# Champii/raiko

Hardware: AMD Instinct MI355X
Metric: proven RISC-V cycles/sec (higher is better)
Workload: dtype u32 (BabyBear Montgomery)

## Files before the change

### raiko_amd/csrc/internal.hpp

```cpp
#pragma once
#include <hip/hip_runtime.h>

#include <cstring>
#include <map>
#include <memory>
#include <new>
#include <string>
#include <unordered_map>
#include <vector>

#include "../../include/raiko_hip.h"
#include "taps.hpp"
#include "bb.hpp"
#include "ntt_core.hpp"
#include "poseidon2_core.hpp"
#include "params.hpp"

struct rk_ctx {
    int device = 0;
    hipStream_t stream = nullptr;
    bool own_stream = false;
    std::string last_error;

    uint32_t* d_tables = nullptr;
// ... 79 lines not shown
int ntt_reverse_from(rk_ctx* ctx, uint32_t* d_dst, const uint32_t* d_src, size_t size, size_t count, bool fuse_zk_shift);
int ntt_forward(rk_ctx* ctx, uint32_t* d_out, const uint32_t* d_in, size_t in_size, size_t count,
                unsigned expand_bits);
int zk_shift(rk_ctx* ctx, uint32_t* d_io, size_t size, size_t count);
int bit_reverse(rk_ctx* ctx, uint32_t* d_io, size_t size, size_t count);

int hash_rows(rk_ctx* ctx, uint32_t* d_out, const uint32_t* d_matrix, size_t rows, size_t cols);
int hash_fold(rk_ctx* ctx, uint32_t* d_nodes, size_t output_size);
int merkle_build(rk_ctx* ctx, uint32_t* d_nodes, const uint32_t* d_matrix, size_t rows, size_t cols);
int pow_grind(rk_ctx* ctx, const uint32_t* h_cells, unsigned bits, uint32_t* nonce);
int duplex_grind(rk_ctx* ctx, const uint32_t* h_state, const uint32_t* h_input, unsigned n_input, unsigned bits, uint32_t* witness);

int eltwise_add(rk_ctx* ctx, uint32_t* d_out, const uint32_t* a, const uint32_t* b, size_t n);
int eltwise_sum_ext(rk_ctx* ctx, uint32_t* d_out, const uint32_t* d_in, size_t count, size_t to_add);
int eltwise_zeroize(rk_ctx* ctx, uint32_t* d_io, size_t n);
int fri_fold(rk_ctx* ctx, uint32_t* d_out, const uint32_t* d_in, size_t out_count, const bb::Ext& mix);
int fri_fold_evals(rk_ctx* ctx, uint32_t* d_out_ext, const uint32_t* d_in_ext, size_t n_out, const bb::Ext& beta);
int gather_sample(rk_ctx* ctx, uint32_t* d_dst, const uint32_t* d_src, size_t idx, size_t size, size_t stride);
int gather_rows(rk_ctx* ctx, uint32_t* d_dst, const uint32_t* d_matrix, size_t rows, size_t cols,
                const uint32_t* d_idx, size_t n_idx);
int gather_digests(rk_ctx* ctx, uint32_t* d_dst, const uint32_t* d_nodes, const uint32_t* d_idx, size_t n_idx);
struct GatherJob {
    const uint32_t* matrix;
    const uint32_t* nodes;
    uint64_t rows, cols, idx_off, dst_off;
    uint32_t n, path_len;
};
int gather_many(rk_ctx* ctx, uint32_t* d_dst, const uint32_t* d_idx, const GatherJob* d_jobs, const GatherJob* h_jobs, size_t n_jobs);
int ext_powers(rk_ctx* ctx, uint32_t* d_pw_ext, const bb::Ext& x, size_t n, bool bit_reversed);
int ext_powers_many(rk_ctx* ctx, uint32_t* d_pw_ext, const bb::Ext* h_pts, size_t n_pts, size_t n, bool bit_reversed);
int bit_reverse_ext(rk_ctx* ctx, uint32_t* d_io_ext, size_t size, size_t count);
constexpr size_t HASH_FOLD_TOP_MAX = 4096;
int hash_fold_top(rk_ctx* ctx, uint32_t* d_nodes, size_t top_output_size);
int eval_dot(rk_ctx* ctx, uint32_t* d_out_ext, const uint32_t* d_coeffs, size_t size, const uint32_t* d_which,
             const uint32_t* d_pw_ext, const uint32_t* d_pw_sel, size_t eval_count);
int mix_poly_coeffs(rk_ctx* ctx, uint32_t* d_out_ext, const bb::Ext& mix_start, const bb::Ext& mix,
                    const uint32_t* d_in, const uint32_t* h_combos, size_t input_size, size_t count);
int poly_divide(rk_ctx* ctx, uint32_t* d_poly_ext, size_t count, const bb::Ext& z, bb::Ext* h_rem);
int poly_divide_many(rk_ctx* ctx, uint32_t* d_base_ext, size_t count, const size_t* h_offsets, const bb::Ext* h_z,
                     size_t n_items, bb::Ext* h_rems, uint32_t* d_rems = nullptr);
int prefix_products(rk_ctx* ctx, uint32_t* d_io_ext, size_t count);
int scatter(rk_ctx* ctx, uint32_t* d_into, size_t into_words, const uint32_t* h_index, size_t n_cycles,
            const uint32_t* h_offsets, const uint32_t* h_values);
int program_eval_check(const rk_program* prog, const rk_circuit_view* view, const uint32_t poly_mix[4], uint32_t* d_check);
int program_poly_ext(const rk_program* prog, uint32_t wm, const uint32_t poly_mix[4], const uint32_t* eval_u_ext, size_t n_taps,
                     const uint32_t* globals, uint32_t n_globals, const uint32_t* mix, uint32_t n_mix, uint32_t out_ext[4]);
int pcs_coset_lde_rows(rk_ctx* ctx, uint32_t* d_out, const uint32_t* d_in, size_t h, size_t w, uint32_t** keep_cols = nullptr);
int pcs_cols_to_rows_bitrev(rk_ctx* ctx, uint32_t* d_out, const uint32_t* d_cols, size_t H, size_t w);
int pcs_eval_at(rk_ctx* ctx, uint32_t* d_out_ext, const uint32_t* d_lde, size_t H, size_t w, const uint32_t* h_points, size_t n_points,
                bool cols = false);
int pcs_reduce_openings(rk_ctx* ctx, uint32_t* d_ro_ext, const uint32_t* d_lde, size_t H, size_t w, size_t n_points,
                        const uint32_t* h_points, const uint32_t* h_ys, const bb::Ext& alpha, uint64_t alpha_offset, bool cols = false);
int pcs_coset_lde_cols(rk_ctx* ctx, uint32_t* d_cols, const uint32_t* d_in, size_t h, size_t w);
int ext_sub_at(rk_ctx* ctx, uint32_t* d_ext, const uint32_t* h_idx, const bb::Ext* h_delta, size_t n);
void p3_release_pools();

struct CodeKey {
    uint32_t fp[4];
    uint32_t po2, cols, blowup_log2, queries;
    uint32_t root27m, shiftm;
    uint32_t p2[8];
    bool operator==(const CodeKey& o) const { return std::memcmp(this, &o, sizeof(CodeKey)) == 0; }
};
struct CodeEntry {
    CodeKey key{};
    int device = 0;
    uint32_t* coeffs = nullptr;
    uint32_t* evaluated = nullptr;
    uint32_t* nodes = nullptr;
    std::vector<uint32_t> top;
// ... 16 lines not shown
```

### raiko_amd/csrc/kernels_poly.hip

```cpp
#include "internal.hpp"

#include <algorithm>
#include <cstring>

namespace {

using bb::Ext;
constexpr int TPB = 256;

inline unsigned grid_for(size_t n, unsigned cap = 16384) {
    size_t b = (n + TPB - 1) / TPB;
    if (b < 1) b = 1;
    return (unsigned)(b > cap ? cap : b);
}

__device__ __forceinline__ Ext load_ext(const uint32_t* p) {
    uint4 v = *reinterpret_cast<const uint4*>(p);
    return Ext{{v.x, v.y, v.z, v.w}};
}
__device__ __forceinline__ void store_ext(uint32_t* p, const Ext& e) {
    *reinterpret_cast<uint4*>(p) = make_uint4(e.c[0], e.c[1], e.c[2], e.c[3]);
}

__global__ void add_kernel(uint32_t* out, const uint32_t* a, const uint32_t* b, size_t n) {
    size_t i = (size_t)blockIdx.x * blockDim.x + threadIdx.x, st = (size_t)gridDim.x * blockDim.x;
    for (; i < n; i += st) out[i] = bb::add(a[i], b[i]);
}
__global__ void zeroize_kernel(uint32_t* io, size_t n) {
    size_t i = (size_t)blockIdx.x * blockDim.x + threadIdx.x, st = (size_t)gridDim.x * blockDim.x;
    for (; i < n; i += st)
        if (io[i] == bb::INVALID) io[i] = 0;
}
__global__ void sum_ext_kernel(uint32_t* out, const uint32_t* in, size_t count, size_t to_add) {
    size_t i = (size_t)blockIdx.x * blockDim.x + threadIdx.x, st = (size_t)gridDim.x * blockDim.x;
    for (; i < count; i += st) {
        Ext tot = bb::ext_zero();
        for (size_t j = 0; j < to_add; j++) tot = bb::add(tot, load_ext(in + (j * count + i) * 4));
#pragma unroll
        for (int k = 0; k < 4; k++) out[(size_t)k * count + i] = tot.c[k];
    }
}

struct FoldPows {
    Ext p[16];
};
template <int LOG_A>
__global__ void fri_fold_kernel(uint32_t* out, const uint32_t* in, size_t count, FoldPows pw, uint32_t wm) {
    constexpr unsigned A = 1u << LOG_A;
    size_t idx = (size_t)blockIdx.x * blockDim.x + threadIdx.x, st = (size_t)gridDim.x * blockDim.x;
    for (; idx < count; idx += st) {
        Ext tot = bb::ext_zero();
// ... 65 lines not shown
        store_ext(pw + pos * 4, cur);
        cur = bb::mul(cur, x, wm);
    }
}
__global__ void ext_powers_many_kernel(uint32_t* pw, const Ext* xs, size_t n, unsigned rev_bits, uint32_t wm) {
    size_t t = (size_t)blockIdx.x * blockDim.x + threadIdx.x;
    size_t start = t * PW_CH;
    if (start >= n) return;
    const Ext x = xs[blockIdx.y];
    pw += (size_t)blockIdx.y * n * 4;
    Ext cur = bb::pow(x, (uint64_t)start, wm);
    size_t end = start + PW_CH < n ? start + PW_CH : n;
    for (size_t k = start; k < end; k++) {
        size_t pos = rev_bits ? (size_t)bb::bitrev((uint32_t)k, rev_bits) : k;
        store_ext(pw + pos * 4, cur);
        cur = bb::mul(cur, x, wm);
    }
}
__global__ void bit_reverse_ext_kernel(uint32_t* io, size_t total, size_t size, unsigned bits) {
    size_t idx = (size_t)blockIdx.x * blockDim.x + threadIdx.x, st = (size_t)gridDim.x * blockDim.x;
    for (; idx < total; idx += st) {
        uint32_t pos = (uint32_t)(idx & (size - 1));
        uint32_t rev = bb::bitrev(pos, bits);
        if (pos < rev) {
            size_t other = idx - pos + rev;
            Ext a = load_ext(io + idx * 4), b = load_ext(io + other * 4);
            store_ext(io + idx * 4, b);
            store_ext(io + other * 4, a);
        }
    }
}

constexpr int DOT_BLOCKS = 64;
__global__ __launch_bounds__(TPB) void eval_dot_kernel(uint32_t* __restrict__ partial, const uint32_t* __restrict__ coeffs,
                                                       size_t size, const uint32_t* __restrict__ which,
                                                       const uint32_t* __restrict__ pw, const uint32_t* __restrict__ sel) {
    __shared__ uint32_t red[TPB * 4];
    size_t e = blockIdx.y;
    const uint32_t* c = coeffs + (size_t)which[e] * size;
    const uint32_t* p = pw + (size_t)sel[e] * size * 4;
    Ext acc = bb::ext_zero();
    constexpr size_t STEP = (size_t)DOT_BLOCKS * TPB;
    size_t k = (size_t)blockIdx.x * TPB + threadIdx.x;
    for (; k + 3 * STEP < size; k += 4 * STEP) {
        uint32_t v[4];
        Ext t[4];
#pragma unroll
        for (int u = 0; u < 4; u++) {
            v[u] = c[k + u * STEP];
            t[u] = load_ext(p + (k + u * STEP) * 4);
        }
#pragma unroll
        for (int u = 0; u < 4; u++) acc = bb::add(acc, bb::scale(t[u], v[u]));
    }
    for (; k < size; k += STEP) acc = bb::add(acc, bb::scale(load_ext(p + k * 4), c[k]));
#pragma unroll
    for (int j = 0; j < 4; j++) red[threadIdx.x * 4 + j] = acc.c[j];
    __syncthreads();
    for (int s = TPB / 2; s > 0; s >>= 1) {
        if ((int)threadIdx.x < s) {
#pragma unroll
            for (int j = 0; j < 4; j++)
                red[threadIdx.x * 4 + j] = bb::add(red[threadIdx.x * 4 + j], red[(threadIdx.x + s) * 4 + j]);
        }
        __syncthreads();
    }
    if (threadIdx.x < 4) partial[(e * DOT_BLOCKS + blockIdx.x) * 4 + threadIdx.x] = red[threadIdx.x];
}
__global__ void eval_reduce_kernel(uint32_t* out, const uint32_t* partial, size_t n_eval) {
    size_t i = (size_t)blockIdx.x * blockDim.x + threadIdx.x;
    if (i >= n_eval * 4) return;
    size_t e = i >> 2, j = i & 3;
    uint32_t acc = 0;
    for (int b = 0; b < DOT_BLOCKS; b++) acc = bb::add(acc, partial[(e * DOT_BLOCKS + b) * 4 + j]);
    out[i] = acc;
}

__global__ void mix_kernel(uint32_t* __restrict__ out, const uint32_t* __restrict__ in, size_t count,
                           const uint32_t* __restrict__ slot_combo, const uint32_t* __restrict__ slot_off,
                           const uint32_t* __restrict__ cols, const uint32_t* __restrict__ pows) {
    constexpr unsigned U = 8;
    unsigned slot = blockIdx.y;
    size_t combo = slot_combo[slot];
    unsigned t0 = slot_off[slot], t1 = slot_off[slot + 1];
    size_t idx = (size_t)blockIdx.x * blockDim.x + threadIdx.x, st = (size_t)gridDim.x * blockDim.x;
    for (; idx < count; idx += st) {
        uint32_t* o = out + (combo * count + idx) * 4;
        Ext acc = load_ext(o);
        unsigned t = t0;
        for (; t + U <= t1; t += U) {
            uint32_t v[U];
#pragma unroll
            for (unsigned u = 0; u < U; u++) v[u] = in[(size_t)cols[t + u] * count + idx];
#pragma unroll
            for (unsigned u = 0; u < U; u++) acc = bb::add(acc, bb::scale(load_ext(pows + (size_t)(t + u) * 4), v[u]));
        }
        for (; t < t1; t++) {
            Ext pw = load_ext(pows + (size_t)t * 4);
            acc = bb::add(acc, bb::scale(pw, in[(size_t)cols[t] * count + idx]));
        }
        store_ext(o, acc);
    }
}

constexpr int DIV_CH = 64;
constexpr int DIV_NT = 1024;
constexpr int DIV_GRP = 32;
struct DivItem {
    Ext z, zL;
    unsigned long long off;
    uint32_t wm;
    uint32_t pad_;
};
__global__ void div_tops_kernel(uint32_t* tops, const uint32_t* base, size_t count, size_t nchunks, const DivItem* items) {
    size_t b = (size_t)blockIdx.x * blockDim.x + threadIdx.x;
    if (b >= nchunks) return;
    const DivItem it = items[blockIdx.y];
    const uint32_t* poly = base + it.off * 4;
    size_t start = b * DIV_CH;
    size_t end = start + DIV_CH < count ? start + DIV_CH : count;
    Ext s = bb::ext_zero();
    for (size_t k = end; k-- > start;) s = bb::add(bb::mul(s, it.z, it.wm), load_ext(poly + k * 4));
    store_ext(tops + ((size_t)blockIdx.y * nchunks + b) * 4, s);
}
__global__ __launch_bounds__(DIV_NT) void div_carry_kernel(uint32_t* carry, const uint32_t* tops, size_t nchunks,
                                                           const DivItem* items, uint32_t* rem_out) {
    __shared__ uint32_t seg[DIV_NT * 4];
    __shared__ uint32_t sup[DIV_GRP * 4];
    const unsigned t = threadIdx.x;
    const DivItem it = items[blockIdx.y];
    tops += (size_t)blockIdx.y * nchunks * 4;
    carry += (size_t)blockIdx.y * nchunks * 4;
    const size_t per = (nchunks + DIV_NT - 1) / DIV_NT;
    const size_t s0 = (size_t)t * per, s1 = s0 + per < nchunks ? s0 + per : nchunks;
// ... 156 lines not shown
    }
    return RK_OK;
}
int ext_powers(rk_ctx* ctx, uint32_t* d_pw_ext, const bb::Ext& x, size_t n, bool bit_reversed) {
    if (n == 0) return RK_OK;
    if (bit_reversed && !is_pow2(n)) return RK_ERR_INVALID;
    size_t lanes = (n + PW_CH - 1) / PW_CH;
    KTimer kt(ctx, RK_KCLASS_POLY, (double)n * 16);
    hipLaunchKernelGGL(ext_powers_kernel, dim3((unsigned)((lanes + TPB - 1) / TPB)), dim3(TPB), 0, ctx->stream, d_pw_ext,
                       x, n, bit_reversed ? log2u(n) : 0u, ctx->sys.wm);
    return post_launch(ctx, "ext_powers_kernel");
}
int ext_powers_many(rk_ctx* ctx, uint32_t* d_pw_ext, const bb::Ext* h_pts, size_t n_pts, size_t n, bool bit_reversed) {
    if (n == 0 || n_pts == 0) return RK_OK;
    if ((bit_reversed && !is_pow2(n)) || n_pts > 65535) return RK_ERR_INVALID;
    void* d = nullptr;
    RK_TRY(scratch(ctx, n_pts * 16, &d));
    RK_TRY(upload(ctx, d, h_pts, n_pts * 16));
    size_t lanes = (n + PW_CH - 1) / PW_CH;
    KTimer kt(ctx, RK_KCLASS_POLY, (double)n * 16 * n_pts);
    hipLaunchKernelGGL(ext_powers_many_kernel, dim3((unsigned)((lanes + TPB - 1) / TPB), (unsigned)n_pts), dim3(TPB), 0, ctx->stream,
                       d_pw_ext, (const Ext*)d, n, bit_reversed ? log2u(n) : 0u, ctx->sys.wm);
    return post_launch(ctx, "ext_powers_many_kernel");
}
int bit_reverse_ext(rk_ctx* ctx, uint32_t* d_io_ext, size_t size, size_t count) {
    if (!is_pow2(size) || count == 0) return RK_ERR_INVALID;
    if (size <= 2) return RK_OK;
    size_t total = size * count;
    KTimer kt(ctx, RK_KCLASS_BIT_REVERSE, (double)total * 32);
    hipLaunchKernelGGL(bit_reverse_ext_kernel, dim3(grid_for(total)), dim3(TPB), 0, ctx->stream, d_io_ext, total, size,
                       log2u(size));
    return post_launch(ctx, "bit_reverse_ext_kernel");
}
int eval_dot(rk_ctx* ctx, uint32_t* d_out_ext, const uint32_t* d_coeffs, size_t size, const uint32_t* d_which,
             const uint32_t* d_pw_ext, const uint32_t* d_pw_sel, size_t eval_count) {
    if (eval_count == 0) return RK_OK;
    if (eval_count > 65535) return RK_ERR_INVALID;
    void* partial = nullptr;
    RK_TRY(dev_alloc(ctx, eval_count * DOT_BLOCKS * 16, &partial));
    KTimer kt(ctx, RK_KCLASS_POLY, (double)eval_count * size * 20);
    hipLaunchKernelGGL(eval_dot_kernel, dim3(DOT_BLOCKS, (unsigned)eval_count), dim3(TPB), 0, ctx->stream,
                       (uint32_t*)partial, d_coeffs, size, d_which, d_pw_ext, d_pw_sel);
    int st = post_launch(ctx, "eval_dot_kernel");
    if (st == RK_OK) {
        hipLaunchKernelGGL(eval_reduce_kernel, dim3((unsigned)((eval_count * 4 + TPB - 1) / TPB)), dim3(TPB), 0,
                           ctx->stream, d_out_ext, (const uint32_t*)partial, eval_count);
        st = post_launch(ctx, "eval_reduce_kernel");
    }
    dev_free(ctx, partial);
    return st;
}

int mix_poly_coeffs(rk_ctx* ctx, uint32_t* d_out_ext, const bb::Ext& mix_start, const bb::Ext& mix,
                    const uint32_t* d_in, const uint32_t* h_combos, size_t input_size, size_t count) {
    if (input_size == 0 || count == 0) return RK_OK;
    std::vector<uint32_t> order(input_size);
    for (size_t i = 0; i < input_size; i++) order[i] = (uint32_t)i;
    std::stable_sort(order.begin(), order.end(), [&](uint32_t a, uint32_t b) { return h_combos[a] < h_combos[b]; });
    std::vector<bb::Ext> pw(input_size);
    bb::Ext cur = mix_start;
    for (size_t i = 0; i < input_size; i++) {
        pw[i] = cur;
        cur = bb::mul(cur, mix, ctx->sys.wm);
    }
    std::vector<uint32_t> slot_combo, slot_off, cols(input_size), pows(input_size * 4);
    for (size_t t = 0; t < input_size; t++) {
        uint32_t i = order[t];
        if (t == 0 || h_combos[i] != h_combos[order[t - 1]]) {
            slot_combo.push_back(h_combos[i]);
            slot_off.push_back((uint32_t)t);
        }
        cols[t] = i;
        std::memcpy(&pows[t * 4], pw[i].c, 16);
    }
    slot_off.push_back((uint32_t)input_size);
    size_t n_slots = slot_combo.size();
    size_t o_combo = 0, o_off = o_combo + n_slots, o_cols = o_off + n_slots + 1;
    size_t o_pows = (o_cols + input_size + 3) & ~(size_t)3;
    size_t words = o_pows + input_size * 4;
    std::vector<uint32_t> pack(words, 0);
    std::memcpy(&pack[o_combo], slot_combo.data(), n_slots * 4);
    std::memcpy(&pack[o_off], slot_off.data(), (n_slots + 1) * 4);
    std::memcpy(&pack[o_cols], cols.data(), input_size * 4);
    std::memcpy(&pack[o_pows], pows.data(), input_size * 16);
    void* d = nullptr;
    RK_TRY(scratch(ctx, words * 4, &d));
    RK_TRY(upload(ctx, d, pack.data(), words * 4));
    const uint32_t* dp = (const uint32_t*)d;
    KTimer kt(ctx, RK_KCLASS_POLY, (double)count * (input_size * 4 + n_slots * 32));
    hipLaunchKernelGGL(mix_kernel, dim3(grid_for(count, 4096), (unsigned)n_slots), dim3(TPB), 0, ctx->stream, d_out_ext,
                       d_in, count, dp + o_combo, dp + o_off, dp + o_cols, dp + o_pows);
    return post_launch(ctx, "mix_kernel");
}

int poly_divide_many(rk_ctx* ctx, uint32_t* d_base_ext, size_t count, const size_t* h_offsets, const bb::Ext* h_z,
                     size_t n_items, bb::Ext* h_rems, uint32_t* d_rems) {
    if (count == 0 || n_items == 0 || n_items > 65535) return RK_ERR_INVALID;
    size_t nchunks = (count + DIV_CH - 1) / DIV_CH;
    if (nchunks > (size_t)DIV_NT * 4096) return RK_ERR_INVALID;
    std::vector<DivItem> items(n_items);
    for (size_t i = 0; i < n_items; i++) {
        items[i].z = h_z[i];
        items[i].zL = bb::pow(h_z[i], (uint64_t)DIV_CH, ctx->sys.wm);
        items[i].off = h_offsets[i];
        items[i].wm = ctx->sys.wm;
        items[i].pad_ = 0;
    }
    void* buf = nullptr;
    size_t items_bytes = (n_items * sizeof(DivItem) + 15) & ~(size_t)15;
    RK_TRY(dev_alloc(ctx, items_bytes + n_items * (2 * nchunks + 1) * 16, &buf));
    DivItem* d_items = (DivItem*)buf;
    uint32_t* tops = (uint32_t*)((char*)buf + items_bytes);
    uint32_t* carry = tops + n_items * nchunks * 4;
    uint32_t* rem = carry + n_items * nchunks * 4;
    int st = RK_OK;
    do {
        hipError_t e = hipSuccess;
        st = upload(ctx, d_items, items.data(), n_items * sizeof(DivItem));
        if (st != RK_OK) break;
        unsigned blocks = (unsigned)((nchunks + TPB - 1) / TPB);
        KTimer kt(ctx, RK_KCLASS_POLY, (double)count * 48 * n_items);
        hipLaunchKernelGGL(div_tops_kernel, dim3(blocks, (unsigned)n_items), dim3(TPB), 0, ctx->stream, tops, d_base_ext,
                           count, nchunks, d_items);
        st = post_launch(ctx, "div_tops_kernel");
// ... 94 lines not shown
    bb::Ext b{{beta[0], beta[1], beta[2], beta[3]}};
    return rk::fri_fold_evals(ctx, d_out_ext, d_in_ext, n_out, b);
    RK_GUARD_END
}
int rk_gather_sample(rk_ctx* ctx, uint32_t* d_dst, const uint32_t* d_src, size_t idx, size_t size, size_t stride) {
    RK_GUARD_BEGIN
    if (!ctx || (size && (!d_dst || !d_src))) return RK_ERR_INVALID;
    RK_HIP_TRY(ctx, hipSetDevice(ctx->device));
    return rk::gather_sample(ctx, d_dst, d_src, idx, size, stride);
    RK_GUARD_END
}

int rk_batch_evaluate_any(rk_ctx* ctx, const uint32_t* d_coeffs, size_t poly_count, size_t size,
                          const uint32_t* h_which, const uint32_t* h_xs, size_t eval_count, uint32_t* h_out) {
    RK_GUARD_BEGIN
    if (!ctx || !d_coeffs || !is_pow2(size)) return RK_ERR_INVALID;
    if (eval_count == 0) return RK_OK;
    if (!h_which || !h_xs || !h_out) return RK_ERR_INVALID;
    for (size_t e = 0; e < eval_count; e++)
        if (h_which[e] >= poly_count) return RK_ERR_INVALID;
    RK_HIP_TRY(ctx, hipSetDevice(ctx->device));
    std::vector<bb::Ext> pts;
    std::vector<uint32_t> sel(eval_count);
    for (size_t e = 0; e < eval_count; e++) {
        bb::Ext x{{h_xs[e * 4], h_xs[e * 4 + 1], h_xs[e * 4 + 2], h_xs[e * 4 + 3]}};
        size_t j = 0;
        for (; j < pts.size(); j++)
            if (bb::eq(pts[j], x)) break;
        if (j == pts.size()) pts.push_back(x);
        sel[e] = (uint32_t)j;
    }
    void *d_pw = nullptr, *d_small = nullptr;
    RK_TRY(rk::dev_alloc(ctx, pts.size() * size * 16, &d_pw));
    int st = rk::dev_alloc(ctx, eval_count * (4 + 4 + 16) + 32, &d_small);
    if (st != RK_OK) {
        rk::dev_free(ctx, d_pw);
        return st;
    }
    uint32_t* d_which = (uint32_t*)d_small;
    uint32_t* d_sel = d_which + eval_count;
    uint32_t* d_out = d_sel + eval_count;
    if (((uintptr_t)d_out & 15) != 0) d_out += (16 - ((uintptr_t)d_out & 15)) / 4;
    do {
        hipError_t e1 = hipMemcpyAsync(d_which, h_which, eval_count * 4, hipMemcpyHostToDevice, ctx->stream);
        hipError_t e2 = hipMemcpyAsync(d_sel, sel.data(), eval_count * 4, hipMemcpyHostToDevice, ctx->stream);
        if (e1 != hipSuccess || e2 != hipSuccess) { st = RK_ERR_HIP; ctx->last_error = "evaluate_any h2d"; break; }
        for (size_t j = 0; j < pts.size() && st == RK_OK; j++)
            st = rk::ext_powers(ctx, (uint32_t*)d_pw + j * size * 4, pts[j], size, false);
        if (st != RK_OK) break;
        st = rk::eval_dot(ctx, d_out, d_coeffs, size, d_which, (const uint32_t*)d_pw, d_sel, eval_count);
        if (st != RK_OK) break;
        hipError_t e3 = hipMemcpyAsync(h_out, d_out, eval_count * 16, hipMemcpyDeviceToHost, ctx->stream);
        if (e3 == hipSuccess) e3 = hipStreamSynchronize(ctx->stream);
        if (e3 != hipSuccess) { st = RK_ERR_HIP; ctx->last_error = "evaluate_any d2h"; }
    } while (0);
    if (st != RK_OK) (void)hipStreamSynchronize(ctx->stream);
    rk::dev_free(ctx, d_small);
    rk::dev_free(ctx, d_pw);
    return st;
    RK_GUARD_END
}

int rk_mix_poly_coeffs(rk_ctx* ctx, uint32_t* d_out_ext, const uint32_t mix_start[4], const uint32_t mix[4],
                       const uint32_t* d_in, const uint32_t* h_combos, size_t input_size, size_t count) {
    RK_GUARD_BEGIN
    if (!ctx || !d_out_ext || !d_in || !h_combos || !mix_start || !mix) return RK_ERR_INVALID;
    RK_HIP_TRY(ctx, hipSetDevice(ctx->device));
    bb::Ext ms{{mix_start[0], mix_start[1], mix_start[2], mix_start[3]}};
    bb::Ext mx{{mix[0], mix[1], mix[2], mix[3]}};
    return rk::mix_poly_coeffs(ctx, d_out_ext, ms, mx, d_in, h_combos, input_size, count);
    RK_GUARD_END
}

int rk_poly_divide(rk_ctx* ctx, uint32_t* d_polys_ext, size_t count, const uint32_t z[4], uint32_t* h_rem) {
    RK_GUARD_BEGIN
    if (!ctx || !d_polys_ext || !z || count == 0) return RK_ERR_INVALID;
    RK_HIP_TRY(ctx, hipSetDevice(ctx->device));
    bb::Ext zz{{z[0], z[1], z[2], z[3]}};
    bb::Ext rem;
    RK_TRY(rk::poly_divide(ctx, d_polys_ext, count, zz, &rem));
    if (h_rem) std::memcpy(h_rem, rem.c, 16);
    return RK_OK;
    RK_GUARD_END
}

}
```

### raiko_amd/csrc/prover.hip

```cpp
#include "internal.hpp"

#include <algorithm>
#include <cstring>
#include <memory>

namespace {

using bb::Ext;

struct Transcript {
    p2::Rng rng;
    std::vector<uint32_t> proof;
    explicit Transcript(const p2::Any* kc) : rng(kc) {}
    void write(const uint32_t* w, size_t n) { proof.insert(proof.end(), w, w + n); }
    void commit(const uint32_t* digest) { rng.mix(digest); }
    uint32_t random_elem() { return rng.random_elem(); }
    Ext random_ext() { return rng.random_ext(); }
    uint32_t random_bits(unsigned bits) { return rng.random_bits(bits); }
};

struct DevBuf {
    rk_ctx* ctx = nullptr;
    void* p = nullptr;
    bool borrowed = false;
// ... 459 lines not shown
        if (taps.combo_backs[b] > max_back) max_back = taps.combo_backs[b];
    if (max_back > 64) return RK_ERR_INVALID;
    size_t n_pts = (size_t)max_back + 2;
    std::vector<Ext> pts(n_pts);
    for (uint32_t b = 0; b <= max_back; b++) pts[b] = bb::scale(z, bb::pow(back_one, b));
    pts[max_back + 1] = z_pow;
    std::vector<Ext> all_xs(tot_taps), coeff_u(tot_taps + CHECK_SIZE);
    {
        DevBuf d_pw, d_small;
        RK_TRY(d_pw.alloc(ctx, n_pts * N * 16));
        RK_TRY(rk::ext_powers_many(ctx, d_pw.u32(), pts.data(), n_pts, N, true));
        std::vector<Ext> eval_u(tot_taps + CHECK_SIZE);
        std::vector<uint32_t> which, sel;
        std::vector<size_t> first(5, 0);
        size_t pos = 0;
        uint32_t reg = 0;
        for (uint32_t gid = 0; gid < 3; gid++) {
            for (; reg < taps.n_regs && taps.reg_group[reg] == gid; reg++) {
                uint32_t cb = taps.reg_combo[reg];
                for (uint32_t b = taps.combo_off[cb]; b < taps.combo_off[cb + 1]; b++) {
                    which.push_back(taps.reg_offset[reg]);
                    sel.push_back(taps.combo_backs[b]);
                    all_xs[pos++] = pts[taps.combo_backs[b]];
                }
            }
            first[gid + 1] = pos;
        }
        for (uint32_t i = 0; i < CHECK_SIZE; i++) {
            which.push_back(i);
            sel.push_back(max_back + 1);
        }
        first[4] = pos + CHECK_SIZE;
        const size_t n_ev = first[4];
        RK_TRY(d_small.alloc(ctx, n_ev * (4 + 4 + 16) + 32));
        uint32_t* d_which = d_small.u32();
        uint32_t* d_sel = d_which + n_ev;
        uint32_t* d_out = d_sel + n_ev;
        if (((uintptr_t)d_out & 15) != 0) d_out += (16 - ((uintptr_t)d_out & 15)) / 4;
        RK_TRY(rk::upload(ctx, d_which, which.data(), n_ev * 4));
        RK_TRY(rk::upload(ctx, d_sel, sel.data(), n_ev * 4));
        for (uint32_t gid = 0; gid < 4; gid++) {
            const PolyGroup& pg = gid < 3 ? groups[gid] : check;
            const size_t a = first[gid], n = first[gid + 1] - a;
            if (n) RK_TRY(rk::eval_dot(ctx, d_out + a * 4, pg.coeffs.u32(), N, d_which + a, d_pw.u32(), d_sel + a, n));
        }
        RK_TRY(d2h_sync(ctx, eval_u.data(), d_out, n_ev * 16));
        size_t p = 0;
        for (uint32_t r = 0; r < taps.n_regs; r++) {
            uint32_t cb = taps.reg_combo[r];
            size_t sz = taps.combo_off[cb + 1] - taps.combo_off[cb];
            poly_interpolate(&coeff_u[p], &all_xs[p], &eval_u[p], sz, wm);
            p += sz;
        }
        for (uint32_t i = 0; i < CHECK_SIZE; i++) coeff_u[tot_taps + i] = eval_u[tot_taps + i];
    }
    iop.write((const uint32_t*)coeff_u.data(), coeff_u.size() * 4);
    kc.hash_elems((const uint32_t*)coeff_u.data(), coeff_u.size() * 4, digest);
    iop.commit(digest);

    Ext mix = iop.random_ext();
    const size_t combo_count = taps.n_combos;
    DevBuf combos;
    RK_TRY(combos.alloc(ctx, (combo_count + 1) * N * 16));
    RK_HIP_TRY(ctx, hipMemsetAsync(combos.p, 0, (combo_count + 1) * N * 16, ctx->stream));
    {
        Ext cur_mix = bb::ext_one();
        uint32_t reg = 0;
        std::vector<uint32_t> which;
        for (uint32_t gid = 0; gid < 3; gid++) {
            uint32_t gs = taps.group_size[gid];
            which.assign(gs, 0);
            for (uint32_t i = 0; i < gs; i++, reg++) which[i] = taps.reg_combo[reg];
            RK_TRY(rk::mix_poly_coeffs(ctx, combos.u32(), cur_mix, mix, groups[gid].coeffs.u32(), which.data(), gs, N));
            cur_mix = bb::mul(cur_mix, bb::pow(mix, gs, wm), wm);
        }
        which.assign(CHECK_SIZE, (uint32_t)combo_count);
        RK_TRY(rk::mix_poly_coeffs(ctx, combos.u32(), cur_mix, mix, check.coeffs.u32(), which.data(), CHECK_SIZE, N));
        RK_TRY(rk::bit_reverse_ext(ctx, combos.u32(), N, combo_count + 1));
    }
    DevBuf d_rems;
    {
        std::vector<Ext> delta((combo_count + 1) * (max_back + 2), bb::ext_zero());
        std::vector<uint32_t> delta_idx;
        size_t stride = (size_t)max_back + 2;
        Ext cur = bb::ext_one();
        size_t cur_pos = 0;
        for (uint32_t r = 0; r < taps.n_regs; r++) {
            uint32_t cb = taps.reg_combo[r];
            size_t sz = taps.combo_off[cb + 1] - taps.combo_off[cb];
            if (sz > stride || sz > N) return RK_ERR_INVALID;
            for (size_t i = 0; i < sz; i++)
                delta[cb * stride + i] = bb::add(delta[cb * stride + i], bb::mul(cur, coeff_u[cur_pos + i], wm));
            cur = bb::mul(cur, mix, wm);
            cur_pos += sz;
        }
        for (uint32_t i = 0; i < CHECK_SIZE; i++) {
            delta[combo_count * stride] = bb::add(delta[combo_count * stride], bb::mul(cur, coeff_u[cur_pos++], wm));
            cur = bb::mul(cur, mix, wm);
        }
        std::vector<Ext> dl;
        for (size_t c = 0; c <= combo_count; c++) {
            size_t sz = c < combo_count ? taps.combo_off[c + 1] - taps.combo_off[c] : 1;
            for (size_t i = 0; i < sz; i++) {
                delta_idx.push_back((uint32_t)(c * N + i));
                dl.push_back(delta[c * stride + i]);
            }
        }
        RK_TRY(rk::ext_sub_at(ctx, combos.u32(), delta_idx.data(), dl.data(), dl.size()));
        size_t max_sz = 1;
        for (size_t c = 0; c < combo_count; c++) max_sz = std::max<size_t>(max_sz, taps.combo_off[c + 1] - taps.combo_off[c]);
// ... 141 lines not shown
```

Measured before the change: 49.30 million.

## Batch eval_dot columns per power table and fuse mix passes with lazy reduction

eval_dot now groups evaluations that share the same power table into batches of up to 8 columns. Each power-table load is reused across several coefficient columns, and the four per-group launches become one. mix_poly_coeffs takes all four groups in a single launch that writes fresh combos, which removes the memset and the repeated read-modify-write of the output. Both kernels use a lazy 64-bit accumulator that is folded every four terms, in place of a full modular add per term. The cost is more host-side batch building, higher register pressure from the NB accumulators, and a larger shared-memory reduction.

```diff
diff --git a/raiko_amd/csrc/internal.hpp b/raiko_amd/csrc/internal.hpp
--- a/raiko_amd/csrc/internal.hpp
+++ b/raiko_amd/csrc/internal.hpp
@@ -135,10 +135,19 @@
 int bit_reverse_ext(rk_ctx* ctx, uint32_t* d_io_ext, size_t size, size_t count);
 constexpr size_t HASH_FOLD_TOP_MAX = 4096;
 int hash_fold_top(rk_ctx* ctx, uint32_t* d_nodes, size_t top_output_size);
-int eval_dot(rk_ctx* ctx, uint32_t* d_out_ext, const uint32_t* d_coeffs, size_t size, const uint32_t* d_which,
-             const uint32_t* d_pw_ext, const uint32_t* d_pw_sel, size_t eval_count);
-int mix_poly_coeffs(rk_ctx* ctx, uint32_t* d_out_ext, const bb::Ext& mix_start, const bb::Ext& mix,
-                    const uint32_t* d_in, const uint32_t* h_combos, size_t input_size, size_t count);
+struct EvalSrc {
+    const uint32_t* d_coeffs;
+    size_t n;
+};
+int eval_dot(rk_ctx* ctx, uint32_t* d_out_ext, size_t size, const EvalSrc* srcs, size_t n_srcs, const uint32_t* h_which,
+             const uint32_t* h_sel, const uint32_t* d_pw_ext);
+struct MixSrc {
+    const uint32_t* d_in;
+    const uint32_t* h_combos;
+    size_t n;
+};
+int mix_poly_coeffs(rk_ctx* ctx, uint32_t* d_out_ext, const bb::Ext& mix_start, const bb::Ext& mix, const MixSrc* srcs,
+                    size_t n_srcs, size_t count, size_t fresh_combos);
 int poly_divide(rk_ctx* ctx, uint32_t* d_poly_ext, size_t count, const bb::Ext& z, bb::Ext* h_rem);
 int poly_divide_many(rk_ctx* ctx, uint32_t* d_base_ext, size_t count, const size_t* h_offsets, const bb::Ext* h_z,
                      size_t n_items, bb::Ext* h_rems, uint32_t* d_rems = nullptr);
diff --git a/raiko_amd/csrc/kernels_poly.hip b/raiko_amd/csrc/kernels_poly.hip
--- a/raiko_amd/csrc/kernels_poly.hip
+++ b/raiko_amd/csrc/kernels_poly.hip
@@ -1,4 +1,5 @@
 #include "internal.hpp"
+#include "poly_lazy.hpp"
 
 #include <algorithm>
 #include <cstring>
@@ -17,6 +18,9 @@
 __device__ __forceinline__ Ext load_ext(const uint32_t* p) {
     uint4 v = *reinterpret_cast<const uint4*>(p);
     return Ext{{v.x, v.y, v.z, v.w}};
+}
+__device__ __forceinline__ uint32_t load_global(const uint32_t* p) {
+    return *(const __attribute__((address_space(1))) uint32_t*)p;
 }
 __device__ __forceinline__ void store_ext(uint32_t* p, const Ext& e) {
     *reinterpret_cast<uint4*>(p) = make_uint4(e.c[0], e.c[1], e.c[2], e.c[3]);
@@ -148,40 +152,75 @@
 }
 
 constexpr int DOT_BLOCKS = 64;
-__global__ __launch_bounds__(TPB) void eval_dot_kernel(uint32_t* __restrict__ partial, const uint32_t* __restrict__ coeffs,
-                                                       size_t size, const uint32_t* __restrict__ which,
-                                                       const uint32_t* __restrict__ pw, const uint32_t* __restrict__ sel) {
-    __shared__ uint32_t red[TPB * 4];
-    size_t e = blockIdx.y;
-    const uint32_t* c = coeffs + (size_t)which[e] * size;
-    const uint32_t* p = pw + (size_t)sel[e] * size * 4;
-    Ext acc = bb::ext_zero();
-    constexpr size_t STEP = (size_t)DOT_BLOCKS * TPB;
+constexpr int DOT_BATCH = 8;
+constexpr int DOT_RED_STRIDE = TPB + 8;
+constexpr size_t DOT_STEP = (size_t)DOT_BLOCKS * TPB;
+struct EvalBatch {
+    const uint32_t* col[DOT_BATCH];
+    uint32_t out[DOT_BATCH];
+    uint32_t sel, nb;
+};
+template <int NB>
+__device__ __forceinline__ void eval_dot_body(uint32_t* __restrict__ partial, const EvalBatch* __restrict__ bp,
+                                              const uint32_t* __restrict__ pw, size_t size, uint32_t* red) {
+    const EvalBatch& b = *bp;
+    const uint32_t* p = pw + (size_t)b.sel * size * 4;
+    pl::Acc acc[NB];
+#pragma unroll
+    for (int e = 0; e < NB; e++) acc[e] = pl::zero();
     size_t k = (size_t)blockIdx.x * TPB + threadIdx.x;
-    for (; k + 3 * STEP < size; k += 4 * STEP) {
-        uint32_t v[4];
+    static_assert(pl::FOLD_TERMS == 4, "the trip below is one fold interval");
+    for (; k + 3 * DOT_STEP < size; k += 4 * DOT_STEP) {
         Ext t[4];
+        uint32_t v[4][NB];
 #pragma unroll
         for (int u = 0; u < 4; u++) {
-            v[u] = c[k + u * STEP];
-            t[u] = load_ext(p + (k + u * STEP) * 4);
-        }
-#pragma unroll
-        for (int u = 0; u < 4; u++) acc = bb::add(acc, bb::scale(t[u], v[u]));
-    }
-    for (; k < size; k += STEP) acc = bb::add(acc, bb::scale(load_ext(p + k * 4), c[k]));
-#pragma unroll
-    for (int j = 0; j < 4; j++) red[threadIdx.x * 4 + j] = acc.c[j];
+            t[u] = load_ext(p + (k + u * DOT_STEP) * 4);
+#pragma unroll
+            for (int e = 0; e < NB; e++) v[u][e] = load_global(b.col[e] + k + u * DOT_STEP);
+        }
+#pragma unroll
+        for (int e = 0; e < NB; e++) {
+#pragma unroll
+            for (int u = 0; u < 4; u++) pl::mac(acc[e], v[u][e], t[u]);
+            pl::fold(acc[e]);
+        }
+    }
+    for (; k < size; k += DOT_STEP) {
+        const Ext t = load_ext(p + k * 4);
+#pragma unroll
+        for (int e = 0; e < NB; e++) pl::mac(acc[e], load_global(b.col[e] + k), t);
+    }
+#pragma unroll
+    for (int e = 0; e < NB; e++) {
+        const Ext r = pl::finish(acc[e]);
+#pragma unroll
+        for (int j = 0; j < 4; j++) red[(e * 4 + j) * DOT_RED_STRIDE + threadIdx.x] = r.c[j];
+    }
     __syncthreads();
-    for (int s = TPB / 2; s > 0; s >>= 1) {
-        if ((int)threadIdx.x < s) {
-#pragma unroll
-            for (int j = 0; j < 4; j++)
-                red[threadIdx.x * 4 + j] = bb::add(red[threadIdx.x * 4 + j], red[(threadIdx.x + s) * 4 + j]);
-        }
-        __syncthreads();
-    }
-    if (threadIdx.x < 4) partial[(e * DOT_BLOCKS + blockIdx.x) * 4 + threadIdx.x] = red[threadIdx.x];
+    const unsigned row = threadIdx.x >> 3, s = threadIdx.x & 7;
+    uint32_t val = 0;
+    if (row < NB * 4) {
+        uint64_t sum = 0;
+#pragma unroll 8
+        for (int i = 0; i < TPB / 8; i++) sum += red[row * DOT_RED_STRIDE + i * 8 + s];
+        val = (uint32_t)(sum % bb::P);
+    }
+    val = bb::add(val, __shfl_xor(val, 1));
+    val = bb::add(val, __shfl_xor(val, 2));
+    val = bb::add(val, __shfl_xor(val, 4));
+    if (row < NB * 4 && s == 0) partial[((size_t)bp->out[row >> 2] * DOT_BLOCKS + blockIdx.x) * 4 + (row & 3)] = val;
+}
+__global__ __launch_bounds__(TPB) void eval_dot_kernel(uint32_t* __restrict__ partial, const EvalBatch* __restrict__ batches,
+                                                       size_t size, const uint32_t* __restrict__ pw) {
+    __shared__ uint32_t red[DOT_BATCH * 4 * DOT_RED_STRIDE];
+    const EvalBatch* bp = batches + blockIdx.y;
+    switch (bp->nb) {
+        case 8: eval_dot_body<8>(partial, bp, pw, size, red); break;
+        case 4: eval_dot_body<4>(partial, bp, pw, size, red); break;
+        case 2: eval_dot_body<2>(partial, bp, pw, size, red); break;
+        default: eval_dot_body<1>(partial, bp, pw, size, red); break;
+    }
 }
 __global__ void eval_reduce_kernel(uint32_t* out, const uint32_t* partial, size_t n_eval) {
     size_t i = (size_t)blockIdx.x * blockDim.x + threadIdx.x;
@@ -192,30 +231,39 @@
     out[i] = acc;
 }
 
-__global__ void mix_kernel(uint32_t* __restrict__ out, const uint32_t* __restrict__ in, size_t count,
-                           const uint32_t* __restrict__ slot_combo, const uint32_t* __restrict__ slot_off,
-                           const uint32_t* __restrict__ cols, const uint32_t* __restrict__ pows) {
-    constexpr unsigned U = 8;
+template <bool ACCUM>
+__global__ void mix_kernel(uint32_t* __restrict__ out, size_t count, const uint32_t* __restrict__ slot_combo,
+                           const uint32_t* __restrict__ slot_off, const uint32_t* const* __restrict__ cols,
+                           const uint32_t* __restrict__ pows) {
+    constexpr unsigned U = 2 * pl::FOLD_TERMS;
     unsigned slot = blockIdx.y;
     size_t combo = slot_combo[slot];
     unsigned t0 = slot_off[slot], t1 = slot_off[slot + 1];
     size_t idx = (size_t)blockIdx.x * blockDim.x + threadIdx.x, st = (size_t)gridDim.x * blockDim.x;
     for (; idx < count; idx += st) {
         uint32_t* o = out + (combo * count + idx) * 4;
-        Ext acc = load_ext(o);
+        pl::Acc acc = pl::zero();
         unsigned t = t0;
         for (; t + U <= t1; t += U) {
             uint32_t v[U];
 #pragma unroll
-            for (unsigned u = 0; u < U; u++) v[u] = in[(size_t)cols[t + u] * count + idx];
-#pragma unroll
-            for (unsigned u = 0; u < U; u++) acc = bb::add(acc, bb::scale(load_ext(pows + (size_t)(t + u) * 4), v[u]));
-        }
-        for (; t < t1; t++) {
-            Ext pw = load_ext(pows + (size_t)t * 4);
-            acc = bb::add(acc, bb::scale(pw, in[(size_t)cols[t] * count + idx]));
-        }
-        store_ext(o, acc);
+            for (unsigned u = 0; u < U; u++) v[u] = load_global(cols[t + u] + idx);
+#pragma unroll
+            for (unsigned u = 0; u < U; u++) {
+                pl::mac(acc, v[u], load_ext(pows + (size_t)(t + u) * 4));
+                if ((u + 1) % pl::FOLD_TERMS == 0) pl::fold(acc);
+            }
+        }
+        for (unsigned n = 0; t < t1; t++) {
+            pl::mac(acc, load_global(cols[t] + idx), load_ext(pows + (size_t)t * 4));
+            if (++n == (unsigned)pl::FOLD_TERMS) {
+                pl::fold(acc);
+                n = 0;
+            }
+        }
+        Ext r = pl::finish(acc);
+        if (ACCUM) r = bb::add(load_ext(o), r);
+        store_ext(o, r);
     }
 }
 
@@ -438,15 +486,46 @@
                        log2u(size));
     return post_launch(ctx, "bit_reverse_ext_kernel");
 }
-int eval_dot(rk_ctx* ctx, uint32_t* d_out_ext, const uint32_t* d_coeffs, size_t size, const uint32_t* d_which,
-             const uint32_t* d_pw_ext, const uint32_t* d_pw_sel, size_t eval_count) {
+int eval_dot(rk_ctx* ctx, uint32_t* d_out_ext, size_t size, const EvalSrc* srcs, size_t n_srcs, const uint32_t* h_which,
+             const uint32_t* h_sel, const uint32_t* d_pw_ext) {
+    size_t eval_count = 0;
+    for (size_t g = 0; g < n_srcs; g++) eval_count += srcs[g].n;
     if (eval_count == 0) return RK_OK;
-    if (eval_count > 65535) return RK_ERR_INVALID;
+    if (eval_count > 65535 || size == 0) return RK_ERR_INVALID;
+    std::vector<EvalBatch> batches;
+    std::vector<uint32_t> order;
+    size_t first = 0;
+    for (size_t g = 0; g < n_srcs; first += srcs[g].n, g++) {
+        const size_t n = srcs[g].n;
+        order.resize(n);
+        for (size_t i = 0; i < n; i++) order[i] = (uint32_t)(first + i);
+        std::stable_sort(order.begin(), order.end(), [&](uint32_t a, uint32_t b) { return h_sel[a] < h_sel[b]; });
+        for (size_t i = 0; i < n;) {
+            size_t run = 1;
+            while (i + run < n && h_sel[order[i + run]] == h_sel[order[i]]) run++;
+            for (size_t end = i + run; i < end;) {
+                size_t nb = DOT_BATCH;
+                while (nb > end - i) nb >>= 1;
+                EvalBatch bt{};
+                for (size_t e = 0; e < nb; e++) {
+                    bt.col[e] = srcs[g].d_coeffs + (size_t)h_which[order[i + e]] * size;
+                    bt.out[e] = order[i + e];
+                }
+                bt.sel = h_sel[order[i]];
+                bt.nb = (uint32_t)nb;
+                batches.push_back(bt);
+                i += nb;
+            }
+        }
+    }
+    void* d_batches = nullptr;
+    RK_TRY(scratch(ctx, batches.size() * sizeof(EvalBatch), &d_batches));
+    RK_TRY(upload(ctx, d_batches, batches.data(), batches.size() * sizeof(EvalBatch)));
     void* partial = nullptr;
     RK_TRY(dev_alloc(ctx, eval_count * DOT_BLOCKS * 16, &partial));
-    KTimer kt(ctx, RK_KCLASS_POLY, (double)eval_count * size * 20);
-    hipLaunchKernelGGL(eval_dot_kernel, dim3(DOT_BLOCKS, (unsigned)eval_count), dim3(TPB), 0, ctx->stream,
-                       (uint32_t*)partial, d_coeffs, size, d_which, d_pw_ext, d_pw_sel);
+    KTimer kt(ctx, RK_KCLASS_POLY, (double)size * (eval_count * 4 + batches.size() * 16));
+    hipLaunchKernelGGL(eval_dot_kernel, dim3(DOT_BLOCKS, (unsigned)batches.size()), dim3(TPB), 0, ctx->stream,
+                       (uint32_t*)partial, (const EvalBatch*)d_batches, size, d_pw_ext);
     int st = post_launch(ctx, "eval_dot_kernel");
     if (st == RK_OK) {
         hipLaunchKernelGGL(eval_reduce_kernel, dim3((unsigned)((eval_count * 4 + TPB - 1) / TPB)), dim3(TPB), 0,
@@ -457,45 +536,73 @@
     return st;
 }
 
-int mix_poly_coeffs(rk_ctx* ctx, uint32_t* d_out_ext, const bb::Ext& mix_start, const bb::Ext& mix,
-                    const uint32_t* d_in, const uint32_t* h_combos, size_t input_size, size_t count) {
-    if (input_size == 0 || count == 0) return RK_OK;
+int mix_poly_coeffs(rk_ctx* ctx, uint32_t* d_out_ext, const bb::Ext& mix_start, const bb::Ext& mix, const MixSrc* srcs,
+                    size_t n_srcs, size_t count, size_t fresh_combos) {
+    size_t input_size = 0;
+    for (size_t g = 0; g < n_srcs; g++) input_size += srcs[g].n;
+    if (count == 0 || (input_size == 0 && fresh_combos == 0)) return RK_OK;
+    std::vector<uint32_t> combo_of(input_size);
+    std::vector<const uint32_t*> col_of(input_size);
+    {
+        size_t i = 0;
+        for (size_t g = 0; g < n_srcs; g++)
+            for (size_t c = 0; c < srcs[g].n; c++, i++) {
+                combo_of[i] = srcs[g].h_combos[c];
+                col_of[i] = srcs[g].d_in + c * count;
+                if (fresh_combos && combo_of[i] >= fresh_combos) return RK_ERR_INVALID;
+            }
+    }
     std::vector<uint32_t> order(input_size);
     for (size_t i = 0; i < input_size; i++) order[i] = (uint32_t)i;
-    std::stable_sort(order.begin(), order.end(), [&](uint32_t a, uint32_t b) { return h_combos[a] < h_combos[b]; });
+    std::stable_sort(order.begin(), order.end(), [&](uint32_t a, uint32_t b) { return combo_of[a] < combo_of[b]; });
     std::vector<bb::Ext> pw(input_size);
     bb::Ext cur = mix_start;
     for (size_t i = 0; i < input_size; i++) {
         pw[i] = cur;
         cur = bb::mul(cur, mix, ctx->sys.wm);
     }
-    std::vector<uint32_t> slot_combo, slot_off, cols(input_size), pows(input_size * 4);
+    std::vector<uint32_t> slot_combo, slot_off, pows(input_size * 4);
+    std::vector<const uint32_t*> cols(input_size);
+    auto open_slot = [&](uint32_t combo, size_t t) {
+        slot_combo.push_back(combo);
+        slot_off.push_back((uint32_t)t);
+    };
     for (size_t t = 0; t < input_size; t++) {
         uint32_t i = order[t];
-        if (t == 0 || h_combos[i] != h_combos[order[t - 1]]) {
-            slot_combo.push_back(h_combos[i]);
-            slot_off.push_back((uint32_t)t);
-        }
-        cols[t] = i;
+        if (fresh_combos) {
+            while (slot_combo.size() <= combo_of[i]) open_slot((uint32_t)slot_combo.size(), t);
+        } else if (t == 0 || combo_of[i] != combo_of[order[t - 1]]) {
+            open_slot(combo_of[i], t);
+        }
+        cols[t] = col_of[i];
         std::memcpy(&pows[t * 4], pw[i].c, 16);
     }
+    while (slot_combo.size() < fresh_combos) open_slot((uint32_t)slot_combo.size(), input_size);
     slot_off.push_back((uint32_t)input_size);
     size_t n_slots = slot_combo.size();
-    size_t o_combo = 0, o_off = o_combo + n_slots, o_cols = o_off + n_slots + 1;
-    size_t o_pows = (o_cols + input_size + 3) & ~(size_t)3;
-    size_t words = o_pows + input_size * 4;
+    if (n_slots > 65535) return RK_ERR_INVALID;
+    size_t o_cols = 0, o_pows = (o_cols + input_size * 2 + 3) & ~(size_t)3;
+    size_t o_combo = o_pows + input_size * 4, o_off = o_combo + n_slots;
+    size_t words = o_off + n_slots + 1;
     std::vector<uint32_t> pack(words, 0);
+    if (input_size) {
+        std::memcpy(&pack[o_cols], cols.data(), input_size * 8);
+        std::memcpy(&pack[o_pows], pows.data(), input_size * 16);
+    }
     std::memcpy(&pack[o_combo], slot_combo.data(), n_slots * 4);
     std::memcpy(&pack[o_off], slot_off.data(), (n_slots + 1) * 4);
-    std::memcpy(&pack[o_cols], cols.data(), input_size * 4);
-    std::memcpy(&pack[o_pows], pows.data(), input_size * 16);
     void* d = nullptr;
     RK_TRY(scratch(ctx, words * 4, &d));
     RK_TRY(upload(ctx, d, pack.data(), words * 4));
     const uint32_t* dp = (const uint32_t*)d;
-    KTimer kt(ctx, RK_KCLASS_POLY, (double)count * (input_size * 4 + n_slots * 32));
-    hipLaunchKernelGGL(mix_kernel, dim3(grid_for(count, 4096), (unsigned)n_slots), dim3(TPB), 0, ctx->stream, d_out_ext,
-                       d_in, count, dp + o_combo, dp + o_off, dp + o_cols, dp + o_pows);
+    KTimer kt(ctx, RK_KCLASS_POLY, (double)count * (input_size * 4 + n_slots * (fresh_combos ? 16 : 32)));
+    const dim3 grid(grid_for(count, 4096), (unsigned)n_slots), blk(TPB);
+    if (fresh_combos)
+        hipLaunchKernelGGL(mix_kernel<false>, grid, blk, 0, ctx->stream, d_out_ext, count, dp + o_combo, dp + o_off,
+                           (const uint32_t* const*)(dp + o_cols), dp + o_pows);
+    else
+        hipLaunchKernelGGL(mix_kernel<true>, grid, blk, 0, ctx->stream, d_out_ext, count, dp + o_combo, dp + o_off,
+                           (const uint32_t* const*)(dp + o_cols), dp + o_pows);
     return post_launch(ctx, "mix_kernel");
 }
 
@@ -656,23 +763,18 @@
     }
     void *d_pw = nullptr, *d_small = nullptr;
     RK_TRY(rk::dev_alloc(ctx, pts.size() * size * 16, &d_pw));
-    int st = rk::dev_alloc(ctx, eval_count * (4 + 4 + 16) + 32, &d_small);
+    int st = rk::dev_alloc(ctx, eval_count * 16, &d_small);
     if (st != RK_OK) {
         rk::dev_free(ctx, d_pw);
         return st;
     }
-    uint32_t* d_which = (uint32_t*)d_small;
-    uint32_t* d_sel = d_which + eval_count;
-    uint32_t* d_out = d_sel + eval_count;
-    if (((uintptr_t)d_out & 15) != 0) d_out += (16 - ((uintptr_t)d_out & 15)) / 4;
+    uint32_t* d_out = (uint32_t*)d_small;
     do {
-        hipError_t e1 = hipMemcpyAsync(d_which, h_which, eval_count * 4, hipMemcpyHostToDevice, ctx->stream);
-        hipError_t e2 = hipMemcpyAsync(d_sel, sel.data(), eval_count * 4, hipMemcpyHostToDevice, ctx->stream);
-        if (e1 != hipSuccess || e2 != hipSuccess) { st = RK_ERR_HIP; ctx->last_error = "evaluate_any h2d"; break; }
         for (size_t j = 0; j < pts.size() && st == RK_OK; j++)
             st = rk::ext_powers(ctx, (uint32_t*)d_pw + j * size * 4, pts[j], size, false);
         if (st != RK_OK) break;
-        st = rk::eval_dot(ctx, d_out, d_coeffs, size, d_which, (const uint32_t*)d_pw, d_sel, eval_count);
+        const rk::EvalSrc src{d_coeffs, eval_count};
+        st = rk::eval_dot(ctx, d_out, size, &src, 1, h_which, sel.data(), (const uint32_t*)d_pw);
         if (st != RK_OK) break;
         hipError_t e3 = hipMemcpyAsync(h_out, d_out, eval_count * 16, hipMemcpyDeviceToHost, ctx->stream);
         if (e3 == hipSuccess) e3 = hipStreamSynchronize(ctx->stream);
@@ -692,7 +794,9 @@
     RK_HIP_TRY(ctx, hipSetDevice(ctx->device));
     bb::Ext ms{{mix_start[0], mix_start[1], mix_start[2], mix_start[3]}};
     bb::Ext mx{{mix[0], mix[1], mix[2], mix[3]}};
-    return rk::mix_poly_coeffs(ctx, d_out_ext, ms, mx, d_in, h_combos, input_size, count);
+    if (input_size == 0 || count == 0) return RK_OK;
+    const rk::MixSrc src{d_in, h_combos, input_size};
+    return rk::mix_poly_coeffs(ctx, d_out_ext, ms, mx, &src, 1, count, 0);
     RK_GUARD_END
 }
 
diff --git a/raiko_amd/csrc/poly_lazy.hpp b/raiko_amd/csrc/poly_lazy.hpp
--- /dev/null
+++ b/raiko_amd/csrc/poly_lazy.hpp
@@ -0,0 +1,30 @@
+#pragma once
+#include "bb.hpp"
+
+namespace pl {
+
+constexpr int FOLD_TERMS = 4;
+constexpr uint32_t TWO32_MOD_P = 268435454u;
+static_assert((uint64_t)TWO32_MOD_P == ((uint64_t)1 << 32) % bb::P, "2^32 mod p");
+
+struct Acc {
+    uint64_t a[4];
+};
+RK_HD Acc zero() { return Acc{{0, 0, 0, 0}}; }
+RK_HD void mac(Acc& s, uint32_t v, const bb::Ext& m) {
+#pragma unroll
+    for (int j = 0; j < 4; j++) s.a[j] += (uint64_t)v * m.c[j];
+}
+RK_HD uint64_t fold(uint64_t t) { return (uint64_t)(uint32_t)(t >> 32) * TWO32_MOD_P + (uint32_t)t; }
+RK_HD void fold(Acc& s) {
+#pragma unroll
+    for (int j = 0; j < 4; j++) s.a[j] = fold(s.a[j]);
+}
+RK_HD bb::Ext finish(const Acc& s) {
+    bb::Ext r;
+#pragma unroll
+    for (int j = 0; j < 4; j++) r.c[j] = bb::ucanon(bb::uredc64(fold(s.a[j])));
+    return r;
+}
+
+}
diff --git a/raiko_amd/csrc/prover.hip b/raiko_amd/csrc/prover.hip
--- a/raiko_amd/csrc/prover.hip
+++ b/raiko_amd/csrc/prover.hip
@@ -515,18 +515,12 @@
         }
         first[4] = pos + CHECK_SIZE;
         const size_t n_ev = first[4];
-        RK_TRY(d_small.alloc(ctx, n_ev * (4 + 4 + 16) + 32));
-        uint32_t* d_which = d_small.u32();
-        uint32_t* d_sel = d_which + n_ev;
-        uint32_t* d_out = d_sel + n_ev;
-        if (((uintptr_t)d_out & 15) != 0) d_out += (16 - ((uintptr_t)d_out & 15)) / 4;
-        RK_TRY(rk::upload(ctx, d_which, which.data(), n_ev * 4));
-        RK_TRY(rk::upload(ctx, d_sel, sel.data(), n_ev * 4));
-        for (uint32_t gid = 0; gid < 4; gid++) {
-            const PolyGroup& pg = gid < 3 ? groups[gid] : check;
-            const size_t a = first[gid], n = first[gid + 1] - a;
-            if (n) RK_TRY(rk::eval_dot(ctx, d_out + a * 4, pg.coeffs.u32(), N, d_which + a, d_pw.u32(), d_sel + a, n));
-        }
+        RK_TRY(d_small.alloc(ctx, n_ev * 16));
+        uint32_t* d_out = d_small.u32();
+        rk::EvalSrc srcs[4];
+        for (uint32_t gid = 0; gid < 4; gid++)
+            srcs[gid] = rk::EvalSrc{(gid < 3 ? groups[gid] : check).coeffs.u32(), first[gid + 1] - first[gid]};
+        RK_TRY(rk::eval_dot(ctx, d_out, N, srcs, 4, which.data(), sel.data(), d_pw.u32()));
         RK_TRY(d2h_sync(ctx, eval_u.data(), d_out, n_ev * 16));
         size_t p = 0;
         for (uint32_t r = 0; r < taps.n_regs; r++) {
@@ -545,20 +539,18 @@
     const size_t combo_count = taps.n_combos;
     DevBuf combos;
     RK_TRY(combos.alloc(ctx, (combo_count + 1) * N * 16));
-    RK_HIP_TRY(ctx, hipMemsetAsync(combos.p, 0, (combo_count + 1) * N * 16, ctx->stream));
     {
-        Ext cur_mix = bb::ext_one();
-        uint32_t reg = 0;
-        std::vector<uint32_t> which;
-        for (uint32_t gid = 0; gid < 3; gid++) {
-            uint32_t gs = taps.group_size[gid];
-            which.assign(gs, 0);
-            for (uint32_t i = 0; i < gs; i++, reg++) which[i] = taps.reg_combo[reg];
-            RK_TRY(rk::mix_poly_coeffs(ctx, combos.u32(), cur_mix, mix, groups[gid].coeffs.u32(), which.data(), gs, N));
-            cur_mix = bb::mul(cur_mix, bb::pow(mix, gs, wm), wm);
-        }
-        which.assign(CHECK_SIZE, (uint32_t)combo_count);
-        RK_TRY(rk::mix_poly_coeffs(ctx, combos.u32(), cur_mix, mix, check.coeffs.u32(), which.data(), CHECK_SIZE, N));
+        std::vector<uint32_t> which(taps.n_regs + CHECK_SIZE, (uint32_t)combo_count);
+        for (uint32_t r = 0; r < taps.n_regs; r++) which[r] = taps.reg_combo[r];
+        rk::MixSrc srcs[4];
+        size_t at = 0;
+        for (uint32_t gid = 0; gid < 4; gid++) {
+            const size_t n = gid < 3 ? taps.group_size[gid] : CHECK_SIZE;
+            srcs[gid] = rk::MixSrc{(gid < 3 ? groups[gid] : check).coeffs.u32(), which.data() + at, n};
+            at += n;
+        }
+        if (at != which.size()) return RK_ERR_INVALID;
+        RK_TRY(rk::mix_poly_coeffs(ctx, combos.u32(), bb::ext_one(), mix, srcs, 4, N, combo_count + 1));
         RK_TRY(rk::bit_reverse_ext(ctx, combos.u32(), N, combo_count + 1));
     }
     DevBuf d_rems;
```

Measured after the change: 50.53 million, median of 6. 1.03x the previous value.
